# NVIDIA/retinanet-examples

Hardware: AMD Instinct MI355X
Metric: images/sec end-to-end (incl. decode+NMS), RN50FPN 800px bs=8 (higher is better)
Workload: dtype bf16; 1 GPU; ResNet50FPN bf16 inference, bs=8 per GPU at 800x1280, HIP decode x5 + NMS; global_batch=8, parallelism=replicas x1 (no data-path collective), entry=Model.forward (eval), postproc=fused

## Files before the change

include/odtk_hip.h:

```cpp
#ifndef ODTK_HIP_H
#define ODTK_HIP_H

#include <stddef.h>
#include <stdint.h>

#ifdef __cplusplus
extern "C" {
#endif

#define ODTK_OK                0
#define ODTK_ERR_INVALID      -1
#define ODTK_ERR_WORKSPACE    -2
#define ODTK_ERR_HIP          -3
#define ODTK_ERR_UNSUPPORTED  -4

#define ODTK_MAX_LEVELS    6
#define ODTK_MAX_ANCHORS   32
#define ODTK_ATSS_MAX_TOPK 16
#define ODTK_MAX_TOP_N     16384
#define ODTK_MAX_NMS_COUNT 7680
#define ODTK_MAX_NMS_COUNT_SCRATCH (1 << 22)
#define ODTK_MAX_NMS_DETECTIONS 2048

#define ODTK_F32   0
// ... 145 lines not shown
  int32_t enabled;
  int32_t flip;
} odtk_rotation_t;
int odtk_augment_images_ex(int batch_size, const odtk_image_t *images, const odtk_augment_t *augments, const odtk_rotation_t *rotations,
                           const void *src, size_t src_bytes, const int32_t *tables, size_t tables_len, const void *norm_table, void *out,
                           int height, int width, int dtype, void *workspace, size_t workspace_bytes, void *stream);
int odtk_gemm_init(const char *hipblaslt_path);
size_t odtk_gemm_plan_export(char *text, size_t capacity);
int odtk_gemm_plan_import(const char *text);
int odtk_gemm_plan_pin_misses(void);
#define ODTK_GEMM_ORIGIN_TIMED   0
#define ODTK_GEMM_ORIGIN_PINNED  1
#define ODTK_GEMM_ORIGIN_CAPTURE 2
int odtk_debug_gemm_candidates(size_t m, int n, int k, int dtype, int relu, int residual, size_t workspace_size,
                               int *indices, int capacity);
void odtk_gemm_plan_clear(void);
int odtk_gemm_last_solution(int *origin);
int odtk_gemm_bias_act(void *y, const void *x, const void *w, const float *bias, const void *residual,
                       size_t m, int n, int k, int dtype, int relu,
                       void *workspace, size_t workspace_size, void *stream);
int odtk_bottleneck_seam(void *out, void *z, const void *y2, const void *skip, const void *w3, const float *b3, const void *w1,
                         const float *b1, size_t m, int c_in, int c_mid, int c_next, int dtype, void *stream);

int odtk_snap_to_anchors(int batch_size, const float *targets, int n_max, const float *anchors,
                         int num_anchors, int num_classes, int height, int width, int stride,
                         float iou_background, float iou_foreground,
                         float *cls_target, float *box_target, float *depth, void *stream);

typedef struct odtk_snap_level {
  const float *anchors;
  float *cls_target;
  float *box_target;
  float *depth;
  int32_t height, width, stride, pad_;
} odtk_snap_level_t;
int odtk_snap_to_anchors_levels(int batch_size, const float *targets, int n_max, int n_levels,
                                const odtk_snap_level_t *levels, int num_anchors, int num_classes,
                                float iou_background, float iou_foreground, void *stream);

int odtk_atss_assign_levels(int batch_size, const float *targets, int n_max, int n_levels,
                            const odtk_snap_level_t *levels, int num_anchors, int num_classes, int topk,
                            void *workspace, size_t workspace_size, void *stream);

struct odtk_loss_level;
int odtk_tal_assign_levels(int batch_size, const float *targets, int n_max, int n_levels,
                           const odtk_snap_level_t *levels, const struct odtk_loss_level *heads,
// ... 67 lines not shown
                                     void *workspace, size_t workspace_size, void *stream);
int odtk_quality_loss_levels_backward(int n_levels, const odtk_loss_level_t *levels, const float *const *anchors, int batch_size,
                                      int num_anchors, int num_classes, int dtype, int kind, float alpha, float gamma,
                                      const float *grad_sums, void *stream);

#define ODTK_KERNEL_PREFILTER 0
#define ODTK_KERNEL_SELECT    1
#define ODTK_KERNEL_NMS       2
#define ODTK_KERNEL_IOU       3
#define ODTK_KERNEL_EPILOGUE  4
#define ODTK_KERNEL_TARGETS   5
#define ODTK_KERNEL_GEMM      6
#define ODTK_KERNEL_LOSS      7
#define ODTK_KERNEL_SELHIST   8
#define ODTK_KERNEL_SELFILTER 9
#define ODTK_KERNEL_NMS_ORDER 10
#define ODTK_KERNEL_NMS_MATRIX 11
#define ODTK_KERNEL_POOL      12
#define ODTK_KERNEL_UPSAMPLE  13
#define ODTK_KERNEL_STEM_PACK 14
#define ODTK_KERNEL_LOSS_REDUCE 15
#define ODTK_KERNEL_ATSS_STATS 16
#define ODTK_KERNEL_SEAM      17
#define ODTK_KERNEL_COUNT     18
int odtk_profile_enable(int on);
int odtk_debug_set_trace(void *device_buffer);
int odtk_debug_loss_tuning(int which, int fp32_heads, int threads, int blocks_per_cu, int unroll, int box_blocks);
int odtk_debug_loss_layout(int which, int fp32_heads, int per_wave, int window, int box_rows);
int odtk_debug_loss_tuning_get(int which, int fp32_heads, int out[7]);
#define ODTK_LOSS_FORM_DEFAULT 1
int odtk_debug_loss_form(int form);
int odtk_debug_loss_form_get(void);
int odtk_profile_collect(double total_ms[ODTK_KERNEL_COUNT], int launches[ODTK_KERNEL_COUNT]);

#ifdef __cplusplus
}
#endif
#endif
```

retinanet-examples_amd/csrc/engine.hip:

```cpp
#include <cstring>

#include "runtime.hpp"
#include "epilogue.hpp"
#include "gemm_lt.hpp"
#include "seam.hpp"

namespace {

template <typename T, bool kRes, bool kRelu>
int bias_act_launch(void *y, const float *bias, const void *res, uint64_t n, uint32_t channels, hipStream_t stream) {
  constexpr int per = T::kPerLoad;
  uint64_t done = 0;
  if (channels % per == 0 && n / per >= 256) {
    const uint32_t vpr = channels / per;
    const uint64_t n_vec = n / per;
    uint32_t g = vpr, m = 256;
    while (m) { const uint32_t r_ = g % m; g = m; m = r_; }
    const uint32_t unit = vpr / g;
    uint64_t blocks = (n_vec + 256ull * 4 - 1) / (256ull * 4);
    if (blocks > 256 * 16) blocks = 256 * 16;
    blocks = (blocks + unit - 1) / unit * unit;
    timed_launch(ODTK_KERNEL_EPILOGUE, odtk::bias_act_kernel<T, kRes, kRelu>, dim3(static_cast<unsigned>(blocks)), dim3(256), 0,
                 stream, y, bias, res, n_vec, vpr);
    done = n_vec * per;
  }
  if (done < n) {
    uint64_t blocks = (n - done + 255) / 256;
    if (blocks > 4096) blocks = 4096;
// ... 32 lines not shown
  return ODTK_OK;
}

template <typename T, int N2>
int seam_launch(const void *y2, const void *skip, const void *w3, const float *b3, const void *w1, const float *b1, void *out, void *z,
                uint64_t m, hipStream_t stream) {
  constexpr size_t lds = odtk::seam_lds_bytes<N2>();
  const int rc = allow_dynamic_lds(reinterpret_cast<const void *>(&odtk::bottleneck_seam_kernel<T, N2>), lds, "bottleneck_seam_kernel LDS");
  if (rc != ODTK_OK) return rc;
  int device = 0, cus = 0;
  ODTK_HIP_TRY(hipGetDevice(&device));
  ODTK_HIP_TRY(hipDeviceGetAttribute(&cus, hipDeviceAttributeMultiprocessorCount, device));
  constexpr uint64_t per_group = odtk::kSeamThreads / 64 * 32;
  uint64_t blocks = (m + per_group - 1) / per_group;
  const uint64_t resident = static_cast<uint64_t>(cus > 0 ? cus : 1) * (160 * 1024 / lds);
  if (blocks > resident) blocks = resident;
  timed_launch(ODTK_KERNEL_SEAM, odtk::bottleneck_seam_kernel<T, N2>, dim3(static_cast<unsigned>(blocks)), dim3(odtk::kSeamThreads), lds, stream,
               static_cast<const uint16_t *>(y2), static_cast<const uint16_t *>(skip), static_cast<const uint16_t *>(w3), b3,
               static_cast<const uint16_t *>(w1), b1, static_cast<uint16_t *>(out), static_cast<uint16_t *>(z), m);
  ODTK_HIP_TRY(hipGetLastError());
  return ODTK_OK;
}

}

extern "C" {

int odtk_bottleneck_seam(void *out, void *z, const void *y2, const void *skip, const void *w3, const float *b3, const void *w1,
                         const float *b1, size_t m, int c_in, int c_mid, int c_next, int dtype, void *stream) {
  if (!out || !z || !y2 || !skip || !w3 || !b3 || !w1 || !b1 || c_in <= 0 || c_mid <= 0 || c_next <= 0) return ODTK_ERR_INVALID;
  if (out == z || out == y2 || out == skip || z == y2 || z == skip) return ODTK_ERR_INVALID;
  if (dtype != ODTK_BF16 && dtype != ODTK_F16) return ODTK_ERR_UNSUPPORTED;
  if (c_in != odtk::kSeamCin || c_mid != odtk::kSeamCmid || (c_next != 64 && c_next != 128)) return ODTK_ERR_UNSUPPORTED;
  if ((reinterpret_cast<uintptr_t>(out) | reinterpret_cast<uintptr_t>(z) | reinterpret_cast<uintptr_t>(y2) | reinterpret_cast<uintptr_t>(skip) |
       reinterpret_cast<uintptr_t>(w3) | reinterpret_cast<uintptr_t>(w1)) & 15u)
    return ODTK_ERR_INVALID;
  if ((reinterpret_cast<uintptr_t>(b3) | reinterpret_cast<uintptr_t>(b1)) & 3u) return ODTK_ERR_INVALID;
  if (m > (1ull << 40)) return ODTK_ERR_INVALID;
  if (m == 0) return ODTK_OK;
  hipStream_t s = static_cast<hipStream_t>(stream);
  if (dtype == ODTK_BF16)
    return c_next == 64 ? seam_launch<odtk::BF16, 64>(y2, skip, w3, b3, w1, b1, out, z, m, s)
                        : seam_launch<odtk::BF16, 128>(y2, skip, w3, b3, w1, b1, out, z, m, s);
  return c_next == 64 ? seam_launch<odtk::F16, 64>(y2, skip, w3, b3, w1, b1, out, z, m, s)
                      : seam_launch<odtk::F16, 128>(y2, skip, w3, b3, w1, b1, out, z, m, s);
}

int odtk_bias_act(void *y, const float *bias, const void *residual, size_t n_pixels, int channels, int dtype,
                  int relu, void *stream) {
// ... 148 lines not shown
```

retinanet-examples_amd/odtk/_C.py:

```python
import ctypes
import threading
import os

import torch

_LIB_PATH = os.environ.get('ODTK_HIP_LIBRARY') or os.path.join(os.path.dirname(os.path.abspath(__file__)), 'libodtk_hip.so')

OK, ERR_INVALID, ERR_WORKSPACE, ERR_HIP, ERR_UNSUPPORTED = 0, -1, -2, -3, -4
F32, BF16, F16 = 0, 1, 2
FLAG_ROTATED, FLAG_LOGITS, FLAG_ROTATED_NMS_FIXED_ANGLE = 1, 2, 4
MAX_LEVELS, MAX_ANCHORS, MAX_TOP_N, MAX_NMS_COUNT, MAX_NMS_COUNT_SCRATCH = 6, 32, 16384, 7680, 1 << 22
MAX_CONCAT_PARTS = 8
MAX_TILES = 64
SOFT_NMS_LINEAR, SOFT_NMS_GAUSSIAN = 1, 2
ATSS_MAX_TOPK = 16
BOX_LOSS_IOU, BOX_LOSS_GIOU, BOX_LOSS_DIOU = 1, 2, 3
BOX_LOSS_KINDS = {'iou': BOX_LOSS_IOU, 'giou': BOX_LOSS_GIOU, 'diou': BOX_LOSS_DIOU}
ROTATED_BOX_LOSS_PROBIOU, ROTATED_BOX_LOSS_KLD = 1, 2
ROTATED_BOX_LOSS_KINDS = {'probiou': ROTATED_BOX_LOSS_PROBIOU, 'kld': ROTATED_BOX_LOSS_KLD}
CLS_LOSS_QFL, CLS_LOSS_VFL = 1, 2
CLS_LOSS_KINDS = {'qfl': CLS_LOSS_QFL, 'vfl': CLS_LOSS_VFL}

_vp = ctypes.c_void_p
_vpp = ctypes.POINTER(ctypes.c_void_p)
# ... 127 lines not shown
    'odtk_augment_images_ex': (ctypes.c_int, [ctypes.c_int, ctypes.POINTER(Image), ctypes.POINTER(Augment), ctypes.POINTER(Rotation), _vp, _sz,
                                              _vp, _sz, _vp, _vp, ctypes.c_int, ctypes.c_int, ctypes.c_int, _vp, _sz, _vp]),
    'odtk_nms_sorted_runs': (ctypes.c_int, [ctypes.c_int, _vpp, _vpp, ctypes.c_int, _sz, ctypes.c_int, _vp, ctypes.c_int, ctypes.c_float,
                                            ctypes.c_uint32, _vp, _sz, _vp]),
    'odtk_soft_nms': (ctypes.c_int, [ctypes.c_int, _vpp, _vpp, ctypes.c_int, _sz, ctypes.c_int, ctypes.c_float, ctypes.c_int,
                                     ctypes.c_float, ctypes.c_float, ctypes.c_uint32, _vp, _sz, _vp]),
    'odtk_box_vote': (ctypes.c_int, [ctypes.c_int, _vpp, _vp, _vp, _sz, ctypes.c_int, ctypes.c_float, ctypes.c_uint32, _vp]),
    'odtk_concat_candidates': (ctypes.c_int, [ctypes.c_int, ctypes.c_int, ctypes.POINTER(Candidates), _vpp, ctypes.c_uint32, _vp]),
    'odtk_tile_images': (ctypes.c_int, [_vp, _vp] + [ctypes.c_int] * 7 + [ctypes.POINTER(Tile), ctypes.c_int, ctypes.c_int, _vp]),
    'odtk_merge_tile_candidates': (ctypes.c_int, [ctypes.c_int, ctypes.POINTER(Tile), _vpp, _vpp, _sz] + [ctypes.c_int] * 6 +
                                   [ctypes.c_float, ctypes.c_uint32, _vp]),
    'odtk_gemm_init': (ctypes.c_int, [ctypes.c_char_p]),
    'odtk_gemm_plan_export': (ctypes.c_size_t, [ctypes.c_char_p, ctypes.c_size_t]),
    'odtk_gemm_plan_import': (ctypes.c_int, [ctypes.c_char_p]),
    'odtk_gemm_plan_pin_misses': (ctypes.c_int, []),
    'odtk_debug_gemm_candidates': (ctypes.c_int, [ctypes.c_size_t] + [ctypes.c_int] * 5 + [ctypes.c_size_t, ctypes.POINTER(ctypes.c_int),
                                                  ctypes.c_int]),
    'odtk_gemm_plan_clear': (None, []),
    'odtk_gemm_last_solution': (ctypes.c_int, [ctypes.POINTER(ctypes.c_int)]),
    'odtk_gemm_bias_act': (ctypes.c_int, [ctypes.c_void_p, ctypes.c_void_p, ctypes.c_void_p, ctypes.c_void_p, ctypes.c_void_p,
                                          ctypes.c_size_t, ctypes.c_int, ctypes.c_int, ctypes.c_int, ctypes.c_int,
                                          ctypes.c_void_p, ctypes.c_size_t, ctypes.c_void_p]),
    'odtk_bottleneck_seam': (ctypes.c_int, [ctypes.c_void_p] * 8 + [ctypes.c_size_t] + [ctypes.c_int] * 4 + [ctypes.c_void_p]),
    'odtk_profile_collect': (ctypes.c_int, [ctypes.POINTER(ctypes.c_double), ctypes.POINTER(ctypes.c_int)]),
}

KERNEL_NAMES = ('prefilter_scan_kernel', 'select_decode_kernel', 'nms_kernel', 'iou_pairs_kernel', 'bias_act_kernel',
                'snap_to_anchors_kernel', 'gemm_bias_act', 'retina_loss_kernel', 'select_hist_kernel', 'select_filter_kernel',
                'nms_first_round_kernel', 'rotated_sup_matrix_kernel', 'bias_act_maxpool_kernel', 'upsample_nearest2x_kernel',
                'stem_pack_kernel', 'loss_reduce_kernel', 'atss_stats_kernel', 'bottleneck_seam_kernel')
traffic_count = False
traffic_bytes = {}


def _count(name, nbytes):
    if traffic_count:
        traffic_bytes[name] = traffic_bytes.get(name, 0) + int(nbytes)


_lib = None


def library():
    global _lib
    if _lib is None:
        if not os.path.isfile(_LIB_PATH):
            raise ImportError('odtk._C: %s is missing -- build the HIP library first '
                              '(python __graft_entry__.py, or make -C retinanet-examples_amd/csrc). '
                              'There is no CPU fallback.' % _LIB_PATH)
        lib = ctypes.CDLL(_LIB_PATH)
        for name, (res, args) in _SIGNATURES.items():
            fn = getattr(lib, name)
            fn.restype = res
# ... 917 lines not shown

def bottleneck_seam(y2, skip, w3, b3, w1, b1):
    if not y2.is_cuda or y2.dim() != 4 or y2.dtype not in (torch.bfloat16, torch.float16):
        raise RuntimeError('bottleneck_seam: y2 must be a 4-d CUDA tensor of bfloat16/float16')
    b, k, h, w = y2.shape
    c, n = w3.shape[0], w1.shape[0]
    for name, wt, rows, cols in (('w3', w3, c, k), ('w1', w1, n, c)):
        if wt.numel() != rows * cols or wt.shape[1] != cols or wt.dtype != y2.dtype or wt.device != y2.device or not (
                wt.is_contiguous() or wt.is_contiguous(memory_format=torch.channels_last)):
            raise RuntimeError('bottleneck_seam: %s must be a dense [%d, %d(, 1, 1)] tensor of y2.dtype' % (name, rows, cols))
    if skip.shape != (b, c, h, w) or skip.dtype != y2.dtype or skip.device != y2.device or not _channels_last(skip, True) \
            or not _channels_last(y2, True):
        raise RuntimeError('bottleneck_seam: y2 and skip must be channels_last, skip [B, %d, H, W] of y2.dtype' % c)
    if not _bias_vector(b3, c) or not _bias_vector(b1, n):
        raise RuntimeError('bottleneck_seam: b3 / b1 must be float32 CUDA vectors of length %d / %d' % (c, n))
    out = torch.empty((b, c, h, w), dtype=y2.dtype, device=y2.device, memory_format=torch.channels_last)
    z = torch.empty((b, n, h, w), dtype=y2.dtype, device=y2.device, memory_format=torch.channels_last)
    _launch(library().odtk_bottleneck_seam, 'bottleneck_seam', y2.device, out.data_ptr(), z.data_ptr(), y2.data_ptr(), skip.data_ptr(),
            w3.data_ptr(), b3.data_ptr(), w1.data_ptr(), b1.data_ptr(), b * h * w, k, c, n, _DTYPES[y2.dtype])
    _count('bottleneck_seam_kernel', (y2.numel() + skip.numel() + out.numel() + z.numel()) * y2.element_size())
    return out, z


_CONV_LIB_PATH = os.path.join(os.path.dirname(os.path.abspath(__file__)), 'libodtk_conv.so')
_conv_lib = []


def conv_library():
    if not _conv_lib:
        lib = None
        if os.path.isfile(_CONV_LIB_PATH) and not os.environ.get('ODTK_NO_CONV_LIBRARY'):
            lib = ctypes.CDLL(_CONV_LIB_PATH)
            lib.odtk_conv_bias_act.restype = ctypes.c_int
            lib.odtk_conv_bias_act.argtypes = [ctypes.c_void_p] * 4 + [ctypes.c_int] * 13 + [ctypes.c_void_p]
            lib.odtk_conv_bias_act_pads.restype = ctypes.c_int
            lib.odtk_conv_bias_act_pads.argtypes = [ctypes.c_void_p] * 4 + [ctypes.c_int] * 15 + [ctypes.c_void_p]
            lib.odtk_conv_bias_act_strided.restype = ctypes.c_int
            lib.odtk_conv_bias_act_strided.argtypes = ([ctypes.c_void_p] * 4 + [ctypes.c_int] * 13 + [ctypes.c_longlong] * 6 +
                                                       [ctypes.c_int] * 2 + [ctypes.c_void_p])
            lib.odtk_conv_last_plan.restype = ctypes.c_char_p
            lib.odtk_conv_last_plan.argtypes = []
            lib.odtk_conv_instance_count.restype = ctypes.c_int
            lib.odtk_conv_instance_count.argtypes = [ctypes.c_int]
            lib.odtk_conv_plan_export.restype = ctypes.c_size_t
            lib.odtk_conv_plan_export.argtypes = [ctypes.c_char_p, ctypes.c_size_t]
            lib.odtk_conv_plan_import.restype = ctypes.c_int
# ... 175 lines not shown
```

retinanet-examples_amd/odtk/fused.py:

```python
import hashlib
import json
import os
import threading

import torch
import torch.nn as nn
import torch.nn.functional as F

from . import _C
from . import box as box_ops
from .backbones.resnet import BasicBlock, Bottleneck


_PLAN_LOCK = threading.Lock()
_TLS = threading.local()


def _planning():
    return getattr(_TLS, 'planning', False)


def _key_str(key):
    kind, shape = ('only', key[1:]) if key and key[0] == 'only' else ('act', key)
    return kind + ':' + 'x'.join(str(int(v)) for v in shape)
# ... 42 lines not shown
    origins = [(0, 0)]
    shelf_x = shapes[0][1] + gutter
    shelf_w, row_y, row_h, cursor = None, 0, 0, shelf_x
    for h, w in shapes[1:]:
        if shelf_w is None:
            shelf_w = w
        elif cursor + w > shelf_x + shelf_w and row_y + row_h + gutter + h <= height:
            row_y, row_h, cursor = row_y + row_h + gutter, 0, shelf_x
        origins.append((row_y, cursor))
        shelf_w = max(shelf_w, cursor + w - shelf_x)
        row_h = max(row_h, h)
        cursor += w + gutter
    return ((max(y + h for (y, _), (h, _) in zip(origins, shapes)), max(x + w for (_, x), (_, w) in zip(origins, shapes))), origins)


def _window(x):
    return (x.dim() == 4 and x.shape[1] > 1 and x.stride(1) == 1 and x.stride(3) >= x.shape[1]
            and all(v % 8 == 0 for v in (x.stride(0), x.stride(2), x.stride(3))))


class _Conv(nn.Module):

    use_conv_library = True
    route_mode = os.environ.get('ODTK_CONV_ROUTE', 'auto')

    def __init__(self, conv, bn=None, relu=False, dtype=torch.bfloat16):
        super().__init__()
        w, b = fold_conv_bn(conv, bn)
        self.register_buffer('weight', w.to(dtype).contiguous(memory_format=torch.channels_last))
        self.register_buffer('bias', b.contiguous())
        self.register_buffer('bias_lp', b.to(dtype).contiguous())
        self.stride, self.padding, self.relu, self.groups = conv.stride, conv.padding, relu, conv.groups
        self.pointwise = (tuple(conv.kernel_size) == (1, 1) and tuple(conv.padding) == (0, 0) and conv.groups == 1
                          and tuple(conv.dilation) == (1, 1))
        self.library_ok = (not self.pointwise and conv.groups == 1 and tuple(conv.dilation) == (1, 1)
                           and dtype in (torch.bfloat16, torch.float16) and w.shape[1] % 8 == 0)
        self.strided_ok = (self.pointwise and tuple(conv.stride) != (1, 1) and dtype in (torch.bfloat16, torch.float16)
                           and w.shape[1] % 8 == 0)
        self.zero_bias = None
        self.learned = {}
        self.route = {}

    def conv_only(self, x):
        if (self.library_ok and _Conv.use_conv_library and x.is_cuda and x.is_contiguous(memory_format=torch.channels_last)
                and _C.conv_available()):
            key = ('only',) + tuple(x.shape)
            if self.zero_bias is None:
                self.zero_bias = torch.zeros_like(self.bias_lp)
            if self._routed(key, 'only', x, self._miopen_only, self._library_only):
                try:
                    return self._library_only(x)
                except RuntimeError:
                    self.route[key] = (False, float('inf'), 0.0)
        return self._miopen_only(x)

    def on_view(self, x, only=False):
        if x.is_contiguous(memory_format=torch.channels_last):
            return self.conv_only(x) if only else self(x)
        if self.library_ok and _Conv.use_conv_library and x.is_cuda and _window(x) and _C.conv_available():
            if only and self.zero_bias is None:
                self.zero_bias = torch.zeros_like(self.bias_lp)
            key = (('only',) + tuple(x.shape)) if only else tuple(x.shape)
            two, one = (self._miopen_only, self._library_only) if only else (self._two_pass, self._one_pass)
            if self._routed(key, 'only' if only else 'act', x, two, one):
                try:
                    return self._library_only(x) if only else self._one_pass(x)
                except RuntimeError:
                    pass
        x = x.contiguous(memory_format=torch.channels_last)
        return self.conv_only(x) if only else self(x)

    def _torch(self, x, residual=None):
        y = F.conv2d(x, self.weight, None, self.stride, self.padding, groups=self.groups) + self.bias.to(x.dtype).view(1, -1, 1, 1)
        if residual is not None:
            y = y + residual
        return (F.relu(y) if self.relu else y).contiguous(memory_format=torch.channels_last)

# ... 32 lines not shown
                times.append(e0.elapsed_time(e1) * 1e3)
            return sorted(times)[2]
        t_two = timed(two)
        try:
            t_one = timed(one)
        except RuntimeError:
            t_one = float('inf')
        return (t_one < t_two, t_one, t_two)

    def forward(self, x, residual=None):
        if not x.is_cuda:
            return self._torch(x, residual)
        if self.pointwise and _C.gemm_available():
            if tuple(self.stride) != (1, 1):
                if (residual is None and self.strided_ok and _Conv.use_conv_library and x.is_cuda
                        and x.is_contiguous(memory_format=torch.channels_last) and _C.conv_available()):
                    if self._routed(tuple(x.shape), 'act', x, self._copy_then_gemm, self._one_pass):
                        try:
                            return self._one_pass(x)
                        except RuntimeError:
                            self.route[tuple(x.shape)] = (False, float('inf'), 0.0)
                return self._copy_then_gemm(x, residual)
            return _C.gemm_bias_act(x, self.weight, self.bias, residual, self.relu)
        if (residual is None and self.library_ok and _Conv.use_conv_library and x.is_cuda
                and x.is_contiguous(memory_format=torch.channels_last) and _C.conv_available()):
            if self._routed(tuple(x.shape), 'act', x, self._two_pass, self._one_pass):
                try:
                    return self._one_pass(x)
                except RuntimeError:
                    self.route[tuple(x.shape)] = (False, float('inf'), 0.0)
        return self._two_pass(x, residual)

    def _routed(self, key, kind, x, two, one):
        route = self.route.get(key)
        if route is None and _Conv.route_mode != 'auto':
            route = self.route[key] = (_Conv.route_mode == 'library', None, None)
        if route is None and _planning() and not torch.cuda.is_current_stream_capturing():
            route = self.route[key] = self._measure(x, two, one)
            self.learned[kind] = route[0]
        if route is None:
            return self.learned.get(kind, False)
        return route[0]

    def conv_then_pool(self, x):
        if not x.is_cuda:
            return F.max_pool2d(self._torch(x), 3, 2, 1)
        y = F.conv2d(x, self.weight, None, self.stride, self.padding, groups=self.groups)
        if y.dtype in (torch.bfloat16, torch.float16) and y.shape[1] % 8 == 0:
            return _C.bias_act_maxpool(y.contiguous(memory_format=torch.channels_last), self.bias, self.relu)
        return F.max_pool2d(_C.bias_act_(y.contiguous(memory_format=torch.channels_last), self.bias, None, self.relu), 3, 2, 1)


class _Block(nn.Module):
# ... 47 lines not shown
        super().__init__()
        if not self.supports(model):
            raise ValueError('FusedRetinaNet supports a single ResNet-FPN backbone')
        fpn = next(iter(model.backbones.values()))
        net = fpn.features
        self.dtype = dtype
        self.model = [model]
        self.stem = _Conv(net.conv1, net.bn1, True, dtype)
        self.stem_s2d = None
        c1 = net.conv1
        if (tuple(c1.kernel_size), tuple(c1.stride), tuple(c1.padding), c1.in_channels, c1.groups) == ((7, 7), (2, 2), (3, 3), 3, 1) \
                and dtype in (torch.bfloat16, torch.float16):
            w = self.stem.weight.float()
            w4 = stem_space_to_depth_weights(w)
            self.register_buffer('stem_w4', w4.to(dtype).contiguous(memory_format=torch.channels_last))
            self.register_buffer('stem_zero_bias', torch.zeros(w.shape[0], dtype=dtype, device=w.device))
            self.stem_s2d = {}
        self.stem_learned = False
        self.layers = nn.ModuleList([nn.ModuleList([_Block(b, dtype) for b in layer])
                                     for layer in (net.layer1, net.layer2, net.layer3, net.layer4)])
        blocks = [b for layer in self.layers for b in layer]
        self._seams = {a: b for a, b in zip(blocks, blocks[1:]) if a.seam_to(b, dtype)}
        self.seam_fusion = os.environ.get('ODTK_SEAM_FUSION', '1') != '0'
        self.outputs = list(net.outputs)
        self.lateral = nn.ModuleList([_Conv(fpn.lateral3, None, False, dtype), _Conv(fpn.lateral4, None, False, dtype),
                                      _Conv(fpn.lateral5, None, False, dtype)])
        self.smooth = nn.ModuleList([_Conv(fpn.smooth3, None, False, dtype), _Conv(fpn.smooth4, None, False, dtype),
                                     _Conv(fpn.smooth5, None, False, dtype)])
        self.pyramid6 = _Conv(fpn.pyramid6, None, False, dtype)
        self.pyramid7 = _Conv(fpn.pyramid7, None, False, dtype)

        def head(seq):
            convs = [m for m in seq if isinstance(m, nn.Conv2d)]
            return nn.ModuleList([_Conv(c, None, i + 1 < len(convs), dtype) for i, c in enumerate(convs)])

        self.cls_head = head(model.cls_head)
        self.box_head = head(model.box_head)
        self.level_streams = True
        self.pyramid_canvas = os.environ.get('ODTK_PYRAMID_CANVAS', '1') != '0'
        self._streams = None
        self.tower_plan = 0
        self._planned = set()
        self._loaded_geometries = set()
        self._plan_file_seen = False
        self.libraries_taken = None
        self.max_plans = 4
        self._graphs = {}
        self._thresholds = {}
        self.max_graphs = 8

    def _stem_direct(self, x):
        x = x.to(self.dtype).contiguous(memory_format=torch.channels_last)
        return self.stem.conv_then_pool(x)

    def _stem_packed(self, x):
        xs = _C.stem_pack(x, self.dtype)
        y = _C.conv_bias_act(xs, self.stem_w4, self.stem_zero_bias, 1, ((2, 1), (2, 1)), False)
        return _C.bias_act_maxpool(y, self.stem.bias, self.stem.relu)

    def _stem(self, x):
        if (self.stem_s2d is not None and _Conv.use_conv_library and x.is_cuda and x.dim() == 4 and x.shape[1] == 3
                and x.shape[2] % 2 == 0 and x.shape[3] % 2 == 0 and x.dtype in _C._DTYPES and _C.conv_available()
                and (x.is_contiguous() or x.is_contiguous(memory_format=torch.channels_last))):
            key = (tuple(x.shape), x.dtype, x.is_contiguous())
            route = self.stem_s2d.get(key)
            if route is None and _Conv.route_mode != 'auto':
                route = self.stem_s2d[key] = (_Conv.route_mode == 'library', None, None)
            if route is None and _planning() and not torch.cuda.is_current_stream_capturing():
                route = self.stem_s2d[key] = self.stem._measure(x, self._stem_direct, self._stem_packed)
                self.stem_learned = route[0]
            if route[0] if route is not None else self.stem_learned:
                try:
# ... 123 lines not shown
                e = torch.cuda.Event()
                e.record(stream)
                done.append(e)
        for i in mine:
            unit(i)
        for e in done:
            main.wait_event(e)
        return [o[0] for o in out], [o[1] for o in out]

    def heads(self, x):
        with torch.autocast(x.device.type, enabled=False):
            return self._towers(self.features(x), True)

    def heads_without_last_bias(self, x):
        with torch.autocast(x.device.type, enabled=False):
            cls, box = self._towers(self.features(x), False)
        return cls, box, self.cls_head[-1].bias, self.box_head[-1].bias

    @torch.no_grad()
    def replay(self, x):
        m = self.model[0]
        bias = self.cls_head[-1].bias
        key = (tuple(x.shape), x.dtype, x.device, x.is_contiguous(memory_format=torch.channels_last),
               m.threshold, m.top_n, m.nms, m.detections, self.level_streams, self.tower_plan, self.pyramid_canvas, self.seam_fusion, bias.data_ptr(), bias._version,
               tuple(sorted(m.soft_nms.items())) if getattr(m, 'soft_nms', None) is not None else None,
               getattr(m, 'box_voting', None))
        if getattr(m, 'tta', None) is not None:
            raise RuntimeError('FusedRetinaNet.replay is not available with Model.tta (two passes of the engine)')
        if getattr(m, 'tile', None) is not None:
            raise RuntimeError('FusedRetinaNet.replay is not available with Model.tile (several passes of the engine)')
        entry = self._graphs.get(key)
        if entry is None:
            static_x = torch.empty_like(x)
            static_x.copy_(x)
            side = torch.cuda.Stream(x.device)
            side.wait_stream(torch.cuda.current_stream(x.device))
            with torch.cuda.stream(side):
                for _ in range(2):
                    self.forward(static_x)
            torch.cuda.current_stream(x.device).wait_stream(side)
            graph = torch.cuda.CUDAGraph()
            with torch.cuda.graph(graph):
                out = self.forward(static_x)
            while len(self._graphs) >= self.max_graphs:
                self._graphs.pop(next(iter(self._graphs)))
            entry = self._graphs[key] = (graph, static_x, out, tuple(self._thresholds.values()))
        graph, static_x, out = entry[:3]
# ... 131 lines not shown
```

Measured before the change: 1319 images/s.

## Add custom MFMA implicit-GEMM kernel for 256-channel 3x3 head tower convs

```diff
diff --git a/include/odtk_hip.h b/include/odtk_hip.h
--- a/include/odtk_hip.h
+++ b/include/odtk_hip.h
@@ -191,6 +191,10 @@
 int odtk_bottleneck_seam(void *out, void *z, const void *y2, const void *skip, const void *w3, const float *b3, const void *w1,
                          const float *b1, size_t m, int c_in, int c_mid, int c_next, int dtype, void *stream);
 
+int odtk_tower_conv3x3(void *y, const void *x, const void *w, const void *bias, int batch_size, int height, int width, int c_in,
+                       int c_out, int dtype, int relu, void *stream);
+int odtk_debug_tower_conv_variant(int variant);
+
 int odtk_snap_to_anchors(int batch_size, const float *targets, int n_max, const float *anchors,
                          int num_anchors, int num_classes, int height, int width, int stride,
                          float iou_background, float iou_foreground,
@@ -304,7 +308,8 @@
 #define ODTK_KERNEL_LOSS_REDUCE 15
 #define ODTK_KERNEL_ATSS_STATS 16
 #define ODTK_KERNEL_SEAM      17
-#define ODTK_KERNEL_COUNT     18
+#define ODTK_KERNEL_TOWER_CONV 18
+#define ODTK_KERNEL_COUNT     19
 int odtk_profile_enable(int on);
 int odtk_debug_set_trace(void *device_buffer);
 int odtk_debug_loss_tuning(int which, int fp32_heads, int threads, int blocks_per_cu, int unroll, int box_blocks);
diff --git a/retinanet-examples_amd/csrc/engine.hip b/retinanet-examples_amd/csrc/engine.hip
--- a/retinanet-examples_amd/csrc/engine.hip
+++ b/retinanet-examples_amd/csrc/engine.hip
@@ -4,6 +4,7 @@
 #include "epilogue.hpp"
 #include "gemm_lt.hpp"
 #include "seam.hpp"
+#include "tower_conv.hpp"
 
 namespace {
 
@@ -82,9 +83,58 @@
   return ODTK_OK;
 }
 
+std::atomic<int> g_tower_variant{1};
+
+template <typename T, bool kRelu, int kForm>
+int tower_conv_launch(void *y, const void *x, const void *w, const void *bias, uint32_t m, uint32_t height, uint32_t width, bool remap,
+                      hipStream_t stream) {
+  const int rc = allow_dynamic_lds(reinterpret_cast<const void *>(&odtk::tower_conv3x3_kernel<T, kRelu, kForm>), odtk::tower::kLdsBytes,
+                                   "tower_conv3x3_kernel LDS");
+  if (rc != ODTK_OK) return rc;
+  const uint32_t tiles = (m + odtk::tower::kTilePixels - 1) / odtk::tower::kTilePixels;
+  timed_launch(ODTK_KERNEL_TOWER_CONV, odtk::tower_conv3x3_kernel<T, kRelu, kForm>, dim3(tiles), dim3(odtk::tower::kThreads),
+               odtk::tower::kLdsBytes, stream, static_cast<const unsigned char *>(x), static_cast<const unsigned char *>(w),
+               static_cast<const uint16_t *>(bias), static_cast<unsigned char *>(y), m, height, width, odtk::fastdiv_make(width),
+               odtk::fastdiv_make(height * width), remap ? 1u : 0u);
+  ODTK_HIP_TRY(hipGetLastError());
+  return ODTK_OK;
+}
+
+template <typename T>
+int tower_conv_typed(void *y, const void *x, const void *w, const void *bias, uint32_t m, uint32_t h, uint32_t wd, bool relu, int variant,
+                     hipStream_t s) {
+  const bool remap = variant & 1;
+  if (variant & 2) return relu ? tower_conv_launch<T, true, 0>(y, x, w, bias, m, h, wd, remap, s) : tower_conv_launch<T, false, 0>(y, x, w, bias, m, h, wd, remap, s);
+  return relu ? tower_conv_launch<T, true, 1>(y, x, w, bias, m, h, wd, remap, s) : tower_conv_launch<T, false, 1>(y, x, w, bias, m, h, wd, remap, s);
+}
+
 }
 
 extern "C" {
+
+int odtk_debug_tower_conv_variant(int variant) {
+  if (variant < -1 || variant > 3) return ODTK_ERR_INVALID;
+  return variant < 0 ? g_tower_variant.load() : g_tower_variant.exchange(variant);
+}
+
+int odtk_tower_conv3x3(void *y, const void *x, const void *w, const void *bias, int batch_size, int height, int width, int c_in, int c_out,
+                       int dtype, int relu, void *stream) {
+  if (!y || !x || !w || !bias || batch_size <= 0 || height <= 0 || width <= 0 || c_in <= 0 || c_out <= 0) return ODTK_ERR_INVALID;
+  if (y == x) return ODTK_ERR_INVALID;
+  if (dtype != ODTK_BF16 && dtype != ODTK_F16) return ODTK_ERR_UNSUPPORTED;
+  if (c_in != static_cast<int>(odtk::tower::kChannels) || c_out != static_cast<int>(odtk::tower::kChannels)) return ODTK_ERR_UNSUPPORTED;
+  if ((reinterpret_cast<uintptr_t>(y) | reinterpret_cast<uintptr_t>(x) | reinterpret_cast<uintptr_t>(w) | reinterpret_cast<uintptr_t>(bias)) & 15u)
+    return ODTK_ERR_INVALID;
+  const uint64_t m = static_cast<uint64_t>(batch_size) * static_cast<uint64_t>(height) * static_cast<uint64_t>(width);
+  if (m * odtk::tower::kPixelBytes >= (1ull << 31)) return ODTK_ERR_UNSUPPORTED;
+  hipStream_t s = static_cast<hipStream_t>(stream);
+  const int variant = g_tower_variant.load(std::memory_order_relaxed);
+  if (dtype == ODTK_BF16)
+    return tower_conv_typed<odtk::BF16>(y, x, w, bias, static_cast<uint32_t>(m), static_cast<uint32_t>(height), static_cast<uint32_t>(width),
+                                        relu != 0, variant, s);
+  return tower_conv_typed<odtk::F16>(y, x, w, bias, static_cast<uint32_t>(m), static_cast<uint32_t>(height), static_cast<uint32_t>(width),
+                                      relu != 0, variant, s);
+}
 
 int odtk_bottleneck_seam(void *out, void *z, const void *y2, const void *skip, const void *w3, const float *b3, const void *w1,
                          const float *b1, size_t m, int c_in, int c_mid, int c_next, int dtype, void *stream) {
diff --git a/retinanet-examples_amd/csrc/tower_conv.hpp b/retinanet-examples_amd/csrc/tower_conv.hpp
--- /dev/null
+++ b/retinanet-examples_amd/csrc/tower_conv.hpp
@@ -0,0 +1,201 @@
+#pragma once
+
+#include "common.hpp"
+#include "seam.hpp"
+#include "tower_conv_layout.hpp"
+
+namespace odtk {
+
+typedef float tower_f32x4 __attribute__((ext_vector_type(4)));
+
+__device__ __attribute__((aligned(16))) uint32_t tower_zero_block[4];
+
+template <typename T>
+__device__ __forceinline__ tower_f32x4 tower_mfma(vuint4 a, vuint4 b, tower_f32x4 c) {
+  if constexpr (std::is_same_v<T, BF16>)
+    return __builtin_amdgcn_mfma_f32_16x16x32_bf16(__builtin_bit_cast(seam_bf16x8, a), __builtin_bit_cast(seam_bf16x8, b), c, 0, 0, 0);
+  else
+    return __builtin_amdgcn_mfma_f32_16x16x32_f16(__builtin_bit_cast(seam_f16x8, a), __builtin_bit_cast(seam_f16x8, b), c, 0, 0, 0);
+}
+
+template <typename T>
+__device__ __forceinline__ seam_f32x16 tower_mfma32(vuint4 a, vuint4 b, seam_f32x16 c) {
+  if constexpr (std::is_same_v<T, BF16>)
+    return __builtin_amdgcn_mfma_f32_32x32x16_bf16(__builtin_bit_cast(seam_bf16x8, a), __builtin_bit_cast(seam_bf16x8, b), c, 0, 0, 0);
+  else
+    return __builtin_amdgcn_mfma_f32_32x32x16_f16(__builtin_bit_cast(seam_f16x8, a), __builtin_bit_cast(seam_f16x8, b), c, 0, 0, 0);
+}
+
+__device__ __forceinline__ void tower_glds16(const unsigned char *src, unsigned char *lds_wave_base) {
+  __builtin_amdgcn_global_load_lds((const __attribute__((address_space(1))) void *)src,
+                                   (__attribute__((address_space(3))) void *)lds_wave_base, 16, 0, 0);
+}
+
+template <typename T, bool kRelu, int kForm>
+__global__ __launch_bounds__(tower::kThreads) void tower_conv3x3_kernel(const unsigned char *__restrict__ x, const unsigned char *__restrict__ w,
+                                                                        const uint16_t *__restrict__ bias, unsigned char *__restrict__ y,
+                                                                        uint32_t m, uint32_t height, uint32_t width, FastDiv by_w,
+                                                                        FastDiv by_hw, uint32_t remap) {
+  using namespace tower;
+  extern __shared__ __attribute__((aligned(1024))) unsigned char tower_lds[];
+
+  const uint32_t tid = threadIdx.x, lane = tid & 63u;
+  const uint32_t wave = __builtin_amdgcn_readfirstlane(tid >> 6);
+  uint32_t tile = blockIdx.x;
+  if (remap) {
+    const uint32_t nwg = gridDim.x, q = nwg >> 3, r = nwg & 7u, xcd = tile & 7u;
+    tile = (xcd < r ? xcd * (q + 1u) : r * (q + 1u) + (xcd - r) * q) + (tile >> 3);
+  }
+
+  const uint32_t chunk_bytes = piece_chunk(tid) * 16u;
+  int32_t a_base[4];
+  uint32_t a_mask[4];
+#pragma unroll
+  for (uint32_t i = 0; i < 4; ++i) {
+    const uint32_t p = tile * kTilePixels + piece_row(i, tid);
+    a_base[i] = 0;
+    a_mask[i] = 0u;
+    if (p < m) {
+      const Pixel px = pixel_of(p, by_w, by_hw);
+      a_base[i] = static_cast<int32_t>(p * kPixelBytes + chunk_bytes);
+      a_mask[i] = tap_mask(px.y, px.x, height, width);
+    }
+  }
+  const unsigned char *w_src = w + static_cast<size_t>(piece_row(0, tid)) * (kTaps * kPixelBytes) + chunk_bytes;
+  const unsigned char *zeros = reinterpret_cast<const unsigned char *>(tower_zero_block);
+
+  auto stage = [&](uint32_t kt, uint32_t buffer) {
+    const uint32_t tap = ktile_tap(kt);
+    const int32_t k_bytes = tap_pixel_offset(tap, width) * static_cast<int32_t>(kPixelBytes) + static_cast<int32_t>(ktile_channel(kt) * 2u);
+    unsigned char *dst = tower_lds + buffer * kBufferBytes;
+#pragma unroll
+    for (uint32_t i = 0; i < 4; ++i) {
+      const unsigned char *src = ((a_mask[i] >> tap) & 1u) ? x + static_cast<ptrdiff_t>(a_base[i] + k_bytes) : zeros;
+      tower_glds16(src, dst + piece_wave_base(i, wave));
+    }
+#pragma unroll
+    for (uint32_t i = 0; i < 4; ++i)
+      tower_glds16(w_src + static_cast<size_t>(i) * 64u * (kTaps * kPixelBytes) + kt * kRowBytes, dst + kOperandBytes + piece_wave_base(i, wave));
+  };
+
+  const uint32_t wr = wave >> 2, wc = wave & 3u;
+  using Acc = std::conditional_t<kForm == 0, tower_f32x4[4][8], seam_f32x16[2][4]>;
+  Acc acc;
+  if constexpr (kForm == 0) {
+#pragma unroll
+    for (int n = 0; n < 4; ++n)
+#pragma unroll
+      for (int b = 0; b < 8; ++b) acc[n][b] = tower_f32x4{0.0f, 0.0f, 0.0f, 0.0f};
+  } else {
+#pragma unroll
+    for (int n = 0; n < 2; ++n)
+#pragma unroll
+      for (int b = 0; b < 4; ++b)
+#pragma unroll
+        for (int e = 0; e < 16; ++e) acc[n][b][e] = 0.0f;
+  }
+  uint32_t f[4];
+  if constexpr (kForm == 0) {
+    f[0] = frag_addr(0, 0, lane); f[1] = frag_addr(0, 1, lane); f[2] = f[3] = 0u;
+  } else {
+#pragma unroll
+    for (uint32_t s = 0; s < 4; ++s) f[s] = frag32_addr(0, s, lane);
+  }
+  const uint32_t x_frag = wr * 128u * kRowBytes, w_frag = kOperandBytes + wc * 64u * kRowBytes;
+
+  auto compute = [&](const unsigned char *buf) {
+    if constexpr (kForm == 0) {
+#pragma unroll
+      for (uint32_t kk = 0; kk < 2; ++kk) {
+        vuint4 wf[4], xf[8];
+#pragma unroll
+        for (uint32_t n = 0; n < 4; ++n) wf[n] = *reinterpret_cast<const vuint4 *>(buf + w_frag + n * 16u * kRowBytes + f[kk]);
+#pragma unroll
+        for (uint32_t b = 0; b < 8; ++b) xf[b] = *reinterpret_cast<const vuint4 *>(buf + x_frag + b * 16u * kRowBytes + f[kk]);
+#pragma unroll
+        for (uint32_t n = 0; n < 4; ++n)
+#pragma unroll
+          for (uint32_t b = 0; b < 8; ++b) acc[n][b] = tower_mfma<T>(wf[n], xf[b], acc[n][b]);
+      }
+    } else {
+#pragma unroll
+      for (uint32_t s = 0; s < 4; ++s) {
+        vuint4 wf[2], xf[4];
+#pragma unroll
+        for (uint32_t n = 0; n < 2; ++n) wf[n] = *reinterpret_cast<const vuint4 *>(buf + w_frag + n * 32u * kRowBytes + f[s]);
+#pragma unroll
+        for (uint32_t b = 0; b < 4; ++b) xf[b] = *reinterpret_cast<const vuint4 *>(buf + x_frag + b * 32u * kRowBytes + f[s]);
+#pragma unroll
+        for (uint32_t n = 0; n < 2; ++n)
+#pragma unroll
+          for (uint32_t b = 0; b < 4; ++b) acc[n][b] = tower_mfma32<T>(wf[n], xf[b], acc[n][b]);
+      }
+    }
+  };
+
+  stage(0, 0);
+#pragma unroll 1
+  for (uint32_t kt = 0; kt < kKTiles; kt += 2) {
+#pragma unroll
+    for (uint32_t half = 0; half < 2; ++half) {
+      asm volatile("s_waitcnt vmcnt(0)" ::: "memory");
+      __syncthreads();
+      if (kt + half + 1 < kKTiles) stage(kt + half + 1, half ^ 1u);
+      compute(tower_lds + half * kBufferBytes);
+    }
+  }
+
+  __syncthreads();
+  if constexpr (kForm == 0) {
+#pragma unroll
+    for (uint32_t n = 0; n < 4; ++n)
+#pragma unroll
+      for (uint32_t b = 0; b < 8; ++b) {
+        const uint32_t at = out_addr(acc_pixel(wr * 8u + b, lane), acc_channel(wc * 4u + n, lane, 0));
+        uint2 v;
+        v.x = seam_pack2<T>(acc[n][b][0], acc[n][b][1]);
+        v.y = seam_pack2<T>(acc[n][b][2], acc[n][b][3]);
+        *reinterpret_cast<uint2 *>(tower_lds + at) = v;
+      }
+  } else {
+#pragma unroll
+    for (uint32_t n = 0; n < 2; ++n)
+#pragma unroll
+      for (uint32_t b = 0; b < 4; ++b)
+#pragma unroll
+        for (uint32_t g = 0; g < 4; ++g) {
+          const uint32_t at = out_addr(acc32_pixel(wr * 4u + b, lane), acc32_channel(wc * 2u + n, lane, 4u * g));
+          uint2 v;
+          v.x = seam_pack2<T>(acc[n][b][4 * g], acc[n][b][4 * g + 1]);
+          v.y = seam_pack2<T>(acc[n][b][4 * g + 2], acc[n][b][4 * g + 3]);
+          *reinterpret_cast<uint2 *>(tower_lds + at) = v;
+        }
+  }
+  __syncthreads();
+  const uint32_t pixel0 = tid >> 5, chunk = out_chunk(pixel0, tid & 31u);
+  float bias8[8];
+  {
+    const vuint4 bv = *reinterpret_cast<const vuint4 *>(bias + chunk * 8u);
+#pragma unroll
+    for (int e = 0; e < 8; ++e) bias8[e] = seam_unpack<T>(bv[e >> 1], e & 1);
+  }
+#pragma unroll 4
+  for (uint32_t it = 0; it < 16; ++it) {
+    const uint32_t pixel = it * 16u + pixel0, p = tile * kTilePixels + pixel;
+    const vuint4 v = *reinterpret_cast<const vuint4 *>(tower_lds + (it * kThreads + tid) * 16u);
+    vuint4 r;
+#pragma unroll
+    for (int d = 0; d < 4; ++d) {
+      float o[2];
+#pragma unroll
+      for (int e = 0; e < 2; ++e) {
+        const float s = seam_unpack<T>(v[d], e) + bias8[2 * d + e];
+        o[e] = kRelu ? (s > 0.0f ? s : (s != s ? s : 0.0f)) : s;
+      }
+      r[d] = seam_pack2<T>(o[0], o[1]);
+    }
+    if (p < m) *reinterpret_cast<vuint4 *>(y + static_cast<size_t>(p) * kPixelBytes + chunk * 16u) = r;
+  }
+}
+
+}
diff --git a/retinanet-examples_amd/csrc/tower_conv_layout.hpp b/retinanet-examples_amd/csrc/tower_conv_layout.hpp
--- /dev/null
+++ b/retinanet-examples_amd/csrc/tower_conv_layout.hpp
@@ -0,0 +1,71 @@
+#pragma once
+
+#include "fastdiv.hpp"
+
+namespace odtk {
+namespace tower {
+
+constexpr uint32_t kThreads = 512;
+constexpr uint32_t kTilePixels = 256, kChannels = 256, kBK = 64, kTaps = 9;
+constexpr uint32_t kKTiles = kTaps * kChannels / kBK;
+constexpr uint32_t kRowBytes = kBK * 2, kOperandBytes = 256 * kRowBytes;
+constexpr uint32_t kBufferBytes = 2 * kOperandBytes;
+constexpr uint32_t kLdsBytes = 2 * kBufferBytes;
+constexpr uint32_t kPixelBytes = kChannels * 2;
+
+ODTK_HD uint32_t swizzle(uint32_t row, uint32_t chunk) { return chunk ^ ((row >> 1) & 7u); }
+
+ODTK_HD uint32_t piece_dst(uint32_t i, uint32_t tid) { return (i * kThreads + tid) * 16u; }
+ODTK_HD uint32_t piece_wave_base(uint32_t i, uint32_t wave) { return (i * kThreads + wave * 64u) * 16u; }
+ODTK_HD uint32_t piece_row(uint32_t i, uint32_t tid) { return i * 64u + (tid >> 3); }
+ODTK_HD uint32_t piece_chunk(uint32_t tid) { return swizzle(tid >> 3, tid & 7u); }
+
+ODTK_HD uint32_t frag_row(uint32_t block, uint32_t lane) { return block * 16u + (lane & 15u); }
+ODTK_HD uint32_t frag_chunk(uint32_t kk, uint32_t lane) { return kk * 4u + (lane >> 4); }
+ODTK_HD uint32_t frag_addr(uint32_t block, uint32_t kk, uint32_t lane) {
+  const uint32_t row = frag_row(block, lane);
+  return row * kRowBytes + (swizzle(row, frag_chunk(kk, lane)) << 4);
+}
+
+ODTK_HD uint32_t frag32_row(uint32_t block, uint32_t lane) { return block * 32u + (lane & 31u); }
+ODTK_HD uint32_t frag32_chunk(uint32_t step, uint32_t lane) { return (step >> 1) * 4u + 2u * (lane >> 5) + (step & 1u); }
+ODTK_HD uint32_t frag32_addr(uint32_t block, uint32_t step, uint32_t lane) {
+  const uint32_t row = frag32_row(block, lane);
+  return row * kRowBytes + (swizzle(row, frag32_chunk(step, lane)) << 4);
+}
+
+ODTK_HD uint32_t ktile_tap(uint32_t kt) { return kt >> 2; }
+ODTK_HD uint32_t ktile_channel(uint32_t kt) { return (kt & 3u) * kBK; }
+ODTK_HD int32_t tap_pixel_offset(uint32_t tap, uint32_t width) {
+  return (static_cast<int32_t>(tap / 3u) - 1) * static_cast<int32_t>(width) + (static_cast<int32_t>(tap % 3u) - 1);
+}
+
+struct Pixel { uint32_t n, y, x; };
+ODTK_HD Pixel pixel_of(uint32_t p, const FastDiv &by_w, const FastDiv &by_hw) {
+  Pixel q;
+  uint32_t rem;
+  q.n = fastdivmod(p, by_hw, &rem);
+  q.y = fastdivmod(rem, by_w, &q.x);
+  return q;
+}
+
+ODTK_HD uint32_t tap_mask(uint32_t y, uint32_t x, uint32_t height, uint32_t width) {
+  const uint32_t rows = (y > 0u ? 1u : 0u) | 2u | (y + 1u < height ? 4u : 0u);
+  const uint32_t cols = (x > 0u ? 1u : 0u) | 2u | (x + 1u < width ? 4u : 0u);
+  uint32_t mask = 0u;
+  for (uint32_t kh = 0; kh < 3u; ++kh)
+    if ((rows >> kh) & 1u) mask |= cols << (3u * kh);
+  return mask;
+}
+
+ODTK_HD uint32_t out_chunk(uint32_t pixel, uint32_t chunk) { return (chunk & ~7u) | ((chunk ^ pixel) & 7u); }
+ODTK_HD uint32_t out_addr(uint32_t pixel, uint32_t channel) {
+  return pixel * kPixelBytes + out_chunk(pixel, channel >> 3) * 16u + (channel & 4u) * 2u;
+}
+ODTK_HD uint32_t acc_channel(uint32_t nb, uint32_t lane, uint32_t reg) { return nb * 16u + (lane >> 4) * 4u + reg; }
+ODTK_HD uint32_t acc_pixel(uint32_t mb, uint32_t lane) { return mb * 16u + (lane & 15u); }
+ODTK_HD uint32_t acc32_channel(uint32_t nb, uint32_t lane, uint32_t reg) { return nb * 32u + (reg & 3u) + 8u * (reg >> 2) + 4u * (lane >> 5); }
+ODTK_HD uint32_t acc32_pixel(uint32_t mb, uint32_t lane) { return mb * 32u + (lane & 31u); }
+
+}
+}
diff --git a/retinanet-examples_amd/odtk/_C.py b/retinanet-examples_amd/odtk/_C.py
--- a/retinanet-examples_amd/odtk/_C.py
+++ b/retinanet-examples_amd/odtk/_C.py
@@ -173,13 +173,15 @@
                                           ctypes.c_size_t, ctypes.c_int, ctypes.c_int, ctypes.c_int, ctypes.c_int,
                                           ctypes.c_void_p, ctypes.c_size_t, ctypes.c_void_p]),
     'odtk_bottleneck_seam': (ctypes.c_int, [ctypes.c_void_p] * 8 + [ctypes.c_size_t] + [ctypes.c_int] * 4 + [ctypes.c_void_p]),
+    'odtk_tower_conv3x3': (ctypes.c_int, [ctypes.c_void_p] * 4 + [ctypes.c_int] * 7 + [ctypes.c_void_p]),
+    'odtk_debug_tower_conv_variant': (ctypes.c_int, [ctypes.c_int]),
     'odtk_profile_collect': (ctypes.c_int, [ctypes.POINTER(ctypes.c_double), ctypes.POINTER(ctypes.c_int)]),
 }
 
 KERNEL_NAMES = ('prefilter_scan_kernel', 'select_decode_kernel', 'nms_kernel', 'iou_pairs_kernel', 'bias_act_kernel',
                 'snap_to_anchors_kernel', 'gemm_bias_act', 'retina_loss_kernel', 'select_hist_kernel', 'select_filter_kernel',
                 'nms_first_round_kernel', 'rotated_sup_matrix_kernel', 'bias_act_maxpool_kernel', 'upsample_nearest2x_kernel',
-                'stem_pack_kernel', 'loss_reduce_kernel', 'atss_stats_kernel', 'bottleneck_seam_kernel')
+                'stem_pack_kernel', 'loss_reduce_kernel', 'atss_stats_kernel', 'bottleneck_seam_kernel', 'tower_conv3x3_kernel')
 traffic_count = False
 traffic_bytes = {}
 
@@ -1143,6 +1145,27 @@
     return out, z
 
 
+def tower_conv3x3(x, weight, bias, relu=True):
+    if not x.is_cuda or x.dim() != 4 or x.dtype not in (torch.bfloat16, torch.float16):
+        raise RuntimeError('tower_conv3x3: x must be a 4-d CUDA tensor of bfloat16/float16')
+    b, c, h, w = x.shape
+    n = weight.shape[0]
+    if (weight.dim() != 4 or tuple(weight.shape[1:]) != (c, 3, 3) or weight.dtype != x.dtype or weight.device != x.device
+            or not weight.is_contiguous(memory_format=torch.channels_last)):
+        raise RuntimeError('tower_conv3x3: weight must be a channels_last [Cout, %d, 3, 3] tensor of x.dtype' % c)
+    if not x.is_contiguous(memory_format=torch.channels_last):
+        raise RuntimeError('tower_conv3x3: x must be channels_last')
+    if bias.dtype != x.dtype or bias.numel() != n or bias.device != x.device or not bias.is_contiguous():
+        raise RuntimeError('tower_conv3x3: bias must be a dense vector of length Cout of x.dtype')
+    y = torch.empty((b, n, h, w), dtype=x.dtype, device=x.device, memory_format=torch.channels_last)
+    if y.numel() == 0:
+        return y
+    _launch(library().odtk_tower_conv3x3, 'tower_conv3x3', x.device, y.data_ptr(), x.data_ptr(), weight.data_ptr(), bias.data_ptr(),
+            b, h, w, c, n, _DTYPES[x.dtype], 1 if relu else 0)
+    _count('tower_conv3x3_kernel', (x.numel() + y.numel()) * x.element_size())
+    return y
+
+
 _CONV_LIB_PATH = os.path.join(os.path.dirname(os.path.abspath(__file__)), 'libodtk_conv.so')
 _conv_lib = []
 
diff --git a/retinanet-examples_amd/odtk/fused.py b/retinanet-examples_amd/odtk/fused.py
--- a/retinanet-examples_amd/odtk/fused.py
+++ b/retinanet-examples_amd/odtk/fused.py
@@ -88,6 +88,8 @@
 class _Conv(nn.Module):
 
     use_conv_library = True
+    tower_conv = os.environ.get('ODTK_TOWER_CONV', '1') != '0'
+    tower_min_pixels = 100000
     route_mode = os.environ.get('ODTK_CONV_ROUTE', 'auto')
 
     def __init__(self, conv, bn=None, relu=False, dtype=torch.bfloat16):
@@ -103,22 +105,36 @@
                            and dtype in (torch.bfloat16, torch.float16) and w.shape[1] % 8 == 0)
         self.strided_ok = (self.pointwise and tuple(conv.stride) != (1, 1) and dtype in (torch.bfloat16, torch.float16)
                            and w.shape[1] % 8 == 0)
+        self.tower_ok = (tuple(w.shape) == (256, 256, 3, 3) and tuple(conv.stride) == (1, 1) and tuple(conv.padding) == (1, 1)
+                         and tuple(conv.dilation) == (1, 1) and conv.groups == 1 and dtype in (torch.bfloat16, torch.float16))
         self.zero_bias = None
         self.learned = {}
         self.route = {}
 
     def conv_only(self, x):
+        library = False
         if (self.library_ok and _Conv.use_conv_library and x.is_cuda and x.is_contiguous(memory_format=torch.channels_last)
                 and _C.conv_available()):
             key = ('only',) + tuple(x.shape)
             if self.zero_bias is None:
                 self.zero_bias = torch.zeros_like(self.bias_lp)
-            if self._routed(key, 'only', x, self._miopen_only, self._library_only):
-                try:
-                    return self._library_only(x)
-                except RuntimeError:
-                    self.route[key] = (False, float('inf'), 0.0)
+            library = self._routed(key, 'only', x, self._miopen_only, self._library_only)
+        if library and self._tower_takes(x):
+            try:
+                return _C.tower_conv3x3(x, self.weight, self.zero_bias, False)
+            except RuntimeError:
+                pass
+        if library:
+            try:
+                return self._library_only(x)
+            except RuntimeError:
+                self.route[key] = (False, float('inf'), 0.0)
         return self._miopen_only(x)
+
+    def _tower_takes(self, x, residual=None):
+        return (self.tower_ok and self.tower_conv and residual is None and x.is_cuda and x.dim() == 4 and x.dtype == self.weight.dtype
+                and x.is_contiguous(memory_format=torch.channels_last)
+                and x.shape[0] * x.shape[2] * x.shape[3] >= self.tower_min_pixels)
 
     def on_view(self, x, only=False):
         if x.is_contiguous(memory_format=torch.channels_last):
@@ -197,13 +213,20 @@
                             self.route[tuple(x.shape)] = (False, float('inf'), 0.0)
                 return self._copy_then_gemm(x, residual)
             return _C.gemm_bias_act(x, self.weight, self.bias, residual, self.relu)
+        library = False
         if (residual is None and self.library_ok and _Conv.use_conv_library and x.is_cuda
                 and x.is_contiguous(memory_format=torch.channels_last) and _C.conv_available()):
-            if self._routed(tuple(x.shape), 'act', x, self._two_pass, self._one_pass):
-                try:
-                    return self._one_pass(x)
-                except RuntimeError:
-                    self.route[tuple(x.shape)] = (False, float('inf'), 0.0)
+            library = self._routed(tuple(x.shape), 'act', x, self._two_pass, self._one_pass)
+        if library and self._tower_takes(x, residual):
+            try:
+                return _C.tower_conv3x3(x, self.weight, self.bias_lp, self.relu)
+            except RuntimeError:
+                pass
+        if library:
+            try:
+                return self._one_pass(x)
+            except RuntimeError:
+                self.route[tuple(x.shape)] = (False, float('inf'), 0.0)
         return self._two_pass(x, residual)
 
     def _routed(self, key, kind, x, two, one):
@@ -297,6 +320,7 @@
         blocks = [b for layer in self.layers for b in layer]
         self._seams = {a: b for a, b in zip(blocks, blocks[1:]) if a.seam_to(b, dtype)}
         self.seam_fusion = os.environ.get('ODTK_SEAM_FUSION', '1') != '0'
+        self._tower_conv = _Conv.tower_conv
         self.outputs = list(net.outputs)
         self.lateral = nn.ModuleList([_Conv(fpn.lateral3, None, False, dtype), _Conv(fpn.lateral4, None, False, dtype),
                                       _Conv(fpn.lateral5, None, False, dtype)])
@@ -323,6 +347,17 @@
         self._graphs = {}
         self._thresholds = {}
         self.max_graphs = 8
+
+    @property
+    def tower_conv(self):
+        return self._tower_conv
+
+    @tower_conv.setter
+    def tower_conv(self, on):
+        self._tower_conv = bool(on)
+        for mod in self.modules():
+            if isinstance(mod, _Conv):
+                mod.tower_conv = self._tower_conv
 
     def _stem_direct(self, x):
         x = x.to(self.dtype).contiguous(memory_format=torch.channels_last)
@@ -492,7 +527,7 @@
         m = self.model[0]
         bias = self.cls_head[-1].bias
         key = (tuple(x.shape), x.dtype, x.device, x.is_contiguous(memory_format=torch.channels_last),
-               m.threshold, m.top_n, m.nms, m.detections, self.level_streams, self.tower_plan, self.pyramid_canvas, self.seam_fusion, bias.data_ptr(), bias._version,
+               m.threshold, m.top_n, m.nms, m.detections, self.level_streams, self.tower_plan, self.pyramid_canvas, self.seam_fusion, self.tower_conv, bias.data_ptr(), bias._version,
                tuple(sorted(m.soft_nms.items())) if getattr(m, 'soft_nms', None) is not None else None,
                getattr(m, 'box_voting', None))
         if getattr(m, 'tta', None) is not None:
```

Result: faster. 1379 images/s, median of 6 (+4.5%).
